# NVlabs/CenterPose

Hardware: NVIDIA H100
Metric: images/sec at 512x512 DLA-34 (dla_34 + DCNv2, 7 heads, decode + PnP) (higher is better)
Workload: dtype tf32x3

## Files before the change

centerpose_b200/csrc/dcn_tma.cu:

```cuda
#include <cuda.h>

#include "common.cuh"
#include "umma_common.cuh"

namespace cp {
namespace {

using namespace umma;

constexpr int DT_BM = 128;
constexpr int DT_THREADS = 512;
constexpr int DT_CS = 16;
constexpr int DT_PH = 8, DT_PW = 16;
constexpr int DT_HALO = 8;
constexpr int DT_SH = DT_PH + 2 * DT_HALO, DT_SW = DT_PW + 2 * DT_HALO;
constexpr uint32_t DT_SLAB_BYTES = DT_SH * DT_SW * DT_CS * 4;
constexpr uint32_t DT_COEF_BYTES = DT_BM * 9 * 16;

struct DcnTmaParams {
  CUtensorMap amap;
  const float* src;
  int srcStride;
  const float* offmask;
  int omStride, mask_is_logit;
// ... 37 lines not shown
    float lh = 0.f, lw = 0.f, mk = 0.f;
    uint32_t pk = 0;
    if (h_im > -1.f && w_im > -1.f && h_im < (float)H && w_im < (float)W) {
      const int h_low = (int)floorf(h_im), w_low = (int)floorf(w_im);
      lh = h_im - (float)h_low;
      lw = w_im - (float)w_low;
      const bool t_ok = h_low >= 0, b_ok = h_low + 1 <= H - 1, l_ok = w_low >= 0, r_ok = w_low + 1 <= W - 1;
      const int hl = t_ok ? h_low : 0, hb = b_ok ? h_low + 1 : H - 1;
      const int wl = l_ok ? w_low : 0, wr = r_ok ? w_low + 1 : W - 1;
      const bool in_slab = (hl >= ys) && (hb < ys + DT_SH) && (wl >= xs) && (wr < xs + DT_SW);
      pk = in_slab ? (uint32_t)((hl - ys) * DT_SW + (wl - xs)) : (uint32_t)((hl << 7) | wl);
      pk |= (uint32_t)(wr - wl) << RB_DX;
      pk |= (uint32_t)(hb - hl) << RB_DY;
      pk |= (uint32_t)((t_ok && l_ok) ? 1 : 0) << (RB_W + 0);
      pk |= (uint32_t)((t_ok && r_ok) ? 1 : 0) << (RB_W + 1);
      pk |= (uint32_t)((b_ok && l_ok) ? 1 : 0) << (RB_W + 2);
      pk |= (uint32_t)((b_ok && r_ok) ? 1 : 0) << (RB_W + 3);
      pk |= (uint32_t)(in_slab ? 1 : 0) << RB_SLAB;
      pk |= 1u << RB_LIVE;
      mk = mm;
    }
    st_shared_v4(dst + (uint32_t)tap * 16u, __float_as_uint(lh), __float_as_uint(lw), __float_as_uint(mk), pk);
  }
}

template <bool X3, int BN>
__global__ void __launch_bounds__(DT_THREADS, 1) dcn_tma_kernel(const __grid_constant__ DcnTmaParams p) {
  extern __shared__ __align__(1024) unsigned char smem[];
  DcnCtl* ctl = reinterpret_cast<DcnCtl*>(smem);
  if (threadIdx.x == 0) griddep_launch_dependents();
  const uint32_t sbase = smem_u32(smem);
  const uint32_t coef0 = sbase + 1024u;
  const uint32_t slabs0 = (coef0 + 2u * DT_COEF_BYTES + 1023u) & ~1023u;
  const uint32_t a_stage = X3 ? 16384u : 8192u;
  const uint32_t atiles0 = slabs0 + 2u * DT_SLAB_BYTES;
  const uint32_t btile_bytes = (uint32_t)BN * 64u * (X3 ? 2u : 1u);
  const uint32_t btiles0 = atiles0 + (uint32_t)p.AH * a_stage;
  const uint32_t drain0 = btiles0 + (uint32_t)p.SB * btile_bytes;

  const int tid = threadIdx.x, warp = tid >> 5, lane = tid & 31;
  const int n_tiles = p.CoutPad / BN;
  const int nslab = p.sps;
  const int KB = nslab * 9;
  const int KB_all = (p.Cin / DT_CS) * 9;
  const int KS_SPLIT = p.ksplit;
  const long long total_tiles = p.total_tiles;

  if (tid == 0) {
    for (int s = 0; s < 2; ++s) {
      mbar_init(smem_u32(&ctl->s_full[s]), 1);
      mbar_init(smem_u32(&ctl->s_empty[s]), 4);
      mbar_init(smem_u32(&ctl->c_full[s]), 4);
      mbar_init(smem_u32(&ctl->c_empty[s]), 4);
    }
    for (int s = 0; s < p.AH; ++s) {
      mbar_init(smem_u32(&ctl->a_full[s]), 4);
      mbar_init(smem_u32(&ctl->a_empty[s]), 2);
    }
    for (int s = 0; s < p.SB; ++s) {
      mbar_init(smem_u32(&ctl->b_full[s]), 1);
      mbar_init(smem_u32(&ctl->b_empty[s]), 2);
    }
    fence_mbar_init();
  }
  __syncthreads();
  if (warp != 1) griddep_wait();

// ... 15 lines not shown
            mbar_arrive_expect_tx(bar, DT_SLAB_BYTES);
            tma_load_4d(slabs0 + (uint32_t)stage * DT_SLAB_BYTES, &p.amap, (s0 + s) * DT_CS, x0 - DT_HALO, y0 - DT_HALO, img,
                        bar);
            if (++stage == 2) {
              stage = 0;
              phase ^= 1u;
            }
          }
        }
      }
      __syncwarp();
    } else if (warp == 1) {
      if (lane == 0) {
        int stage = 0;
        uint32_t phase = 0;
        for (long long tile = blockIdx.x; tile < total_tiles; tile += gridDim.x) {
          const int n_tile = (int)((tile / KS_SPLIT) % n_tiles);
          const unsigned char* wsrc = p.wtiles + ((size_t)n_tile * KB_all + (size_t)(tile % KS_SPLIT) * KB) * btile_bytes;
          for (int kb = 0; kb < KB; ++kb) {
            mbar_wait(smem_u32(&ctl->b_empty[stage]), phase ^ 1u);
            const uint32_t bar = smem_u32(&ctl->b_full[stage]);
            mbar_arrive_expect_tx(bar, btile_bytes);
            bulk_g2s(btiles0 + (uint32_t)stage * btile_bytes, wsrc + (size_t)kb * btile_bytes, btile_bytes, bar);
            if (++stage == p.SB) {
              stage = 0;
              phase ^= 1u;
            }
          }
        }
      }
      __syncwarp();
    }
  } else if (warp >= 8 && warp < 12) {
    const int gt = tid - 256;
    const int row = gt & 127;
    const uint32_t a_row = atiles0 + (uint32_t)(row >> 3) * 512u + (uint32_t)(row & 7) * 64u;
    const uint32_t asw = (uint32_t)(row >> 1) & 3u;
    int ss = 0, cb = 0;
    uint32_t ps = 0, pc = 0;
    uint32_t cnt = 0;
    for (long long tile = blockIdx.x; tile < total_tiles; tile += gridDim.x) {
      const long long m_tile = (tile / KS_SPLIT) / n_tiles;
      const int s0 = (int)(tile % KS_SPLIT) * nslab;
      const int img = (int)(m_tile / p.tiles_per_image);
      mbar_wait(smem_u32(&ctl->c_full[cb]), pc);
      const uint32_t crow = coef0 + (uint32_t)cb * DT_COEF_BYTES + (uint32_t)row * 144u;
      const float* gimg = p.src + (size_t)img * p.H * p.W * p.srcStride;
      int cur = -1;
      uint32_t slab = 0;
      float4 rec_next = ld_shared_v4f(crow);
      for (int kb = 0; kb < KB; ++kb) {
        const int s = kb / 9;
        if (s != cur) {
          if (cur >= 0) {
            __syncwarp();
            if (lane == 0) mbar_arrive(smem_u32(&ctl->s_empty[ss]));
            if (++ss == 2) {
              ss = 0;
              ps ^= 1u;
            }
          }
          mbar_wait(smem_u32(&ctl->s_full[ss]), ps);
          slab = slabs0 + (uint32_t)ss * DT_SLAB_BYTES;
          cur = s;
        }
        const float4 rec = rec_next;
// ... 25 lines not shown
              c2[c] = ld_shared_v4f(b2 ^ ((uint32_t)c << 4));
            }
#pragma unroll
            for (int c = 0; c < 4; ++c) {
              c3[c] = ld_shared_v4f(b3 ^ ((uint32_t)c << 4));
              c4[c] = ld_shared_v4f(b4 ^ ((uint32_t)c << 4));
            }
#pragma unroll
            for (int c = 0; c < 4; ++c) {
              v[c].x = w1 * c1[c].x + w2 * c2[c].x + w3 * c3[c].x + w4 * c4[c].x;
              v[c].y = w1 * c1[c].y + w2 * c2[c].y + w3 * c3[c].y + w4 * c4[c].y;
              v[c].z = w1 * c1[c].z + w2 * c2[c].z + w3 * c3[c].z + w4 * c4[c].z;
              v[c].w = w1 * c1[c].w + w2 * c2[c].w + w3 * c3[c].w + w4 * c4[c].w;
            }
          } else {
            const int hl = (int)((pk >> 7) & 127u), wl = (int)(pk & 127u);
            const float* g = gimg + ((size_t)hl * p.W + wl) * p.srcStride + (s0 + s) * DT_CS;
            const size_t dx = (size_t)((pk >> RB_DX) & 1u) * p.srcStride;
            const size_t dy = (size_t)((pk >> RB_DY) & 1u) * p.W * p.srcStride;
#pragma unroll
            for (int c = 0; c < 4; ++c) {
              const float4 c1 = __ldg(reinterpret_cast<const float4*>(g) + c);
              const float4 c2 = __ldg(reinterpret_cast<const float4*>(g + dx) + c);
              const float4 c3 = __ldg(reinterpret_cast<const float4*>(g + dy) + c);
              const float4 c4 = __ldg(reinterpret_cast<const float4*>(g + dy + dx) + c);
              v[c].x = w1 * c1.x + w2 * c2.x + w3 * c3.x + w4 * c4.x;
              v[c].y = w1 * c1.y + w2 * c2.y + w3 * c3.y + w4 * c4.y;
              v[c].z = w1 * c1.z + w2 * c2.z + w3 * c3.z + w4 * c4.z;
              v[c].w = w1 * c1.w + w2 * c2.w + w3 * c3.w + w4 * c4.w;
            }
          }
        }
        const int sa = (int)(cnt & (uint32_t)(p.AH - 1));
        const uint32_t a_hi = a_row + (uint32_t)sa * a_stage + (asw << 4);
        mbar_wait(smem_u32(&ctl->a_empty[sa]), ((cnt >> (p.AH - 1)) & 1u) ^ 1u);
#pragma unroll
        for (int c = 0; c < 4; ++c) {
          const uint32_t off = (uint32_t)c << 4;
          float4 h;
          h.x = tf32_round(v[c].x);
          h.y = tf32_round(v[c].y);
          h.z = tf32_round(v[c].z);
          h.w = tf32_round(v[c].w);
          st_shared_v4f(a_hi ^ off, h.x, h.y, h.z, h.w);
          if (X3)
            st_shared_v4f((a_hi ^ off) + 8192u, tf32_round(v[c].x - h.x), tf32_round(v[c].y - h.y), tf32_round(v[c].z - h.z),
                          tf32_round(v[c].w - h.w));
        }
        fence_proxy_async_smem();
        __syncwarp();
        if (lane == 0) mbar_arrive(smem_u32(&ctl->a_full[sa]));
        ++cnt;
      }
      __syncwarp();
      if (lane == 0) {
        mbar_arrive(smem_u32(&ctl->s_empty[ss]));
        mbar_arrive(smem_u32(&ctl->c_empty[cb]));
      }
      if (++ss == 2) {
        ss = 0;
        ps ^= 1u;
      }
      if (++cb == 2) {
        cb = 0;
        pc ^= 1u;
      }
    }
  } else {
    asm volatile("setmaxnreg.inc.sync.aligned.u32 168;");
    const int c = warp >= 12 ? 1 : 0, wt = tid & 127;
    float* dstage = reinterpret_cast<float*>(smem + (drain0 - sbase)) + (size_t)c * (DRAIN_STAGE_BYTES / 4);
    EpiParams ep;
    ep.bias = p.bias;
    ep.residual = p.residual;
    ep.resStride = p.resStride;
    ep.relu = p.relu;
    ep.res_after_relu = p.res_after_relu;
    ep.round_tf32 = p.round_tf32;
    ep.out = p.out;
    ep.outStride = p.outStride;
    ep.out_nchw = p.out_nchw;
    ep.Cout = p.Cout;
    ep.CoutPad = p.CoutPad;
    ep.H = p.H;
    ep.W = p.W;
    int cb = 0;
    uint32_t pc = 0;
    auto make_records = [&](long long t) {
      const long long mt = (t / KS_SPLIT) / n_tiles;
      const int im = (int)(mt / p.tiles_per_image);
      const int pt = (int)(mt - (long long)im * p.tiles_per_image);
      const int y0 = (pt / p.tiles_x) * DT_PH, x0 = (pt % p.tiles_x) * DT_PW;
      const int oy = y0 + (wt >> 4), ox = x0 + (wt & 15);
      mbar_wait(smem_u32(&ctl->c_empty[cb]), pc ^ 1u);
      coef_row(p, p.offmask + ((size_t)((size_t)im * p.H + oy) * p.W + ox) * p.omStride, oy, ox, y0 - DT_HALO, x0 - DT_HALO,
               coef0 + (uint32_t)cb * DT_COEF_BYTES + (uint32_t)wt * 144u);
      __syncwarp();
      if (lane == 0) mbar_arrive(smem_u32(&ctl->c_full[cb]));
      if (++cb == 2) {
        cb = 0;
        pc ^= 1u;
      }
    };
    if (c == 0 && (long long)blockIdx.x < total_tiles) make_records(blockIdx.x);
    const uint32_t bar_a_full = smem_u32(&ctl->a_full[0]), bar_a_empty = smem_u32(&ctl->a_empty[0]);
    const uint32_t bar_b_full = smem_u32(&ctl->b_full[0]), bar_b_empty = smem_u32(&ctl->b_empty[0]);
    int sb = 0;
    uint32_t pb = 0, cnt = 0;
    float acc[BN / 2];
    float sums[X3 ? BN / 2 : 1];
#pragma unroll
    for (int j = 0; j < BN / 2; ++j) acc[j] = 0.f;
    for (long long tile = blockIdx.x; tile < total_tiles; tile += gridDim.x) {
      if (c == 0 && tile + gridDim.x < total_tiles) make_records(tile + gridDim.x);
#pragma unroll
      for (int j = 0; j < (X3 ? BN / 2 : 1); ++j) sums[j] = 0.f;
      int gk = 0;
      for (int kbi = 0; kbi < KB; ++kbi, ++cnt) {
        const uint32_t sa = cnt & (uint32_t)(p.AH - 1);
        mbar_wait(bar_a_full + 8u * sa, (cnt >> (p.AH - 1)) & 1u);
        mbar_wait(bar_b_full + 8u * (uint32_t)sb, pb);
        const uint64_t da = make_desc(atiles0 + sa * a_stage + (uint32_t)c * 64u * 64u, DT_CS);
        const uint64_t db = make_desc(btiles0 + (uint32_t)sb * btile_bytes, DT_CS);
        mma_kblock<BN, X3, false, 2>(acc, da, db, 8192u >> 4, ((uint32_t)BN * 64u) >> 4, X3 ? gk == 0 : kbi == 0);
        if (wt == 0) {
          mbar_arrive(bar_a_empty + 8u * sa);
          mbar_arrive(bar_b_empty + 8u * (uint32_t)sb);
        }
        if (++sb == p.SB) {
          sb = 0;
          pb ^= 1u;
        }
        if (X3) {
          if (gk == p.group - 1 || kbi == KB - 1) {
#pragma unroll
            for (int j = 0; j < (X3 ? BN / 2 : 1); ++j) sums[j] += acc[X3 ? j : 0];
            gk = 0;
          } else {
            ++gk;
          }
        }
      }
      const int n_tile = (int)((tile / KS_SPLIT) % n_tiles);
      const long long m_tile = (tile / KS_SPLIT) / n_tiles;
      const int n = (int)(m_tile / p.tiles_per_image);
      const int pt = (int)(m_tile - (long long)n * p.tiles_per_image);
      const int col_end = min(p.Cout, (n_tile + 1) * BN);
      auto fn = [&](int r, int cb0, float (&v)[16]) {
        if (cb0 >= BN) return;
        const int i = c * 64 + r;
        if (KS_SPLIT > 1) {
          float4* part_row = reinterpret_cast<float4*>(p.part) + ((size_t)tile * (BN >> 2) + (cb0 >> 2)) * 128 + i;
#pragma unroll
          for (int q = 0; q < 4; ++q) __stcg(part_row + (size_t)q * 128, make_float4(v[4 * q], v[4 * q + 1], v[4 * q + 2], v[4 * q + 3]));
        } else {
          const int oy = (pt / p.tiles_x) * DT_PH + (i >> 4), ox = (pt % p.tiles_x) * DT_PW + (i & 15);
          const int m = (n * p.H + oy) * p.W + ox;
// ... 28 lines not shown
  if (p.kh != 3 || p.kw != 3 || p.stride != 1 || p.pad != 1) return false;
  if (p.Cin % DT_CS || p.srcStride[0] % 4) return false;
  const int W = p.Win, H = p.Hin;
  if (W > 128 || H > 128 || (W % DT_PW) || (H % DT_PH)) return false;
  return dcn_tma_tile_n(p.CoutPad, x3) != 0;
}

int dcn_tma_encode(const IgemmParams& p, int Bmax, void* map_out) {
  return tma_encode_nhwc_box(p.src[0], p.srcC[0], p.Win, p.Hin, Bmax, p.srcStride[0], DT_CS, DT_SW, DT_SH, 1, map_out);
}

int launch_dcn_tma(const IgemmParams& p, const void* map, const ConvKernel& k, cudaStream_t stream, LaunchInfo* info) {
  const bool x3 = k.x3;
  if (!p.wgt_umma) return fail(CP_ERR_INVALID, "dcn_tma: weight tiles missing");
  if (!dcn_tma_supported(p, x3)) return fail(CP_ERR_INVALID, "dcn_tma: unsupported shape");
  DcnTmaParams q;
  memset(&q, 0, sizeof(q));
  memcpy(&q.amap, map, sizeof(CUtensorMap));
  q.src = p.src[0];
  q.srcStride = p.srcStride[0];
  q.offmask = p.offmask;
  q.omStride = p.omStride;
  q.mask_is_logit = p.mask_is_logit;
  q.B = p.B;
  q.H = p.Hin;
  q.W = p.Win;
  q.Cin = p.Cin;
  q.Cout = p.Cout;
  q.CoutPad = p.CoutPad;
  q.BN = k.BN;
  q.tiles_x = p.Win / DT_PW;
  q.tiles_per_image = q.tiles_x * (p.Hin / DT_PH);
  const long long mn = (long long)q.tiles_per_image * p.B * (p.CoutPad / q.BN);
  const uint32_t a_stage = x3 ? 16384u : 8192u;
  q.group = kX3GroupBlocks * 2;
  const uint32_t btile = (uint32_t)q.BN * 64u * (x3 ? 2u : 1u);
  const size_t budget = 226 * 1024;
  q.AH = 2;
  size_t fixed = 1024 + 2 * (size_t)DT_COEF_BYTES + 1024 + 2 * (size_t)DT_SLAB_BYTES + (size_t)q.AH * a_stage +
                 2 * (size_t)DRAIN_STAGE_BYTES;
  if (fixed + 3 * (size_t)btile > budget) {
    q.AH = 1;
    fixed -= a_stage;
  }
  if (fixed + 2 * (size_t)btile > budget) return fail(CP_ERR_INVALID, "dcn_tma: tile does not fit shared memory");
  q.SB = (int)((budget - fixed) / btile);
  if (q.SB > 8) q.SB = 8;
  q.bias = p.bias;
  q.residual = p.residual;
  q.resStride = p.resStride;
  q.relu = p.relu;
  q.res_after_relu = p.res_after_relu;
  q.out = p.out;
  q.outStride = p.outStride;
  q.out_nchw = p.out_nchw;
  q.round_tf32 = k.round_out;
  q.wtiles = (const unsigned char*)p.wgt_umma;
  const size_t smem = fixed + (size_t)q.SB * btile;
  void (*kern)(DcnTmaParams) = nullptr;
  switch (q.BN) {
    case 16: kern = x3 ? dcn_tma_kernel<true, 16> : dcn_tma_kernel<false, 16>; break;
    case 32: kern = x3 ? dcn_tma_kernel<true, 32> : dcn_tma_kernel<false, 32>; break;
    case 64: kern = x3 ? dcn_tma_kernel<true, 64> : dcn_tma_kernel<false, 64>; break;
    case 128: kern = x3 ? dcn_tma_kernel<true, 128> : dcn_tma_kernel<false, 128>; break;
    default: return fail(CP_ERR_INVALID, "dcn_tma: unsupported N tile");
  }
  static PerDevice<bool, 8> configured;
// ... 30 lines not shown
```

centerpose_b200/csrc/igemm_umma.cu:

```cuda
#include "common.cuh"
#include "umma_common.cuh"

namespace cp {
namespace {

constexpr int UM_BM = 128;
constexpr int UM_PROD_WARPS = 8;
constexpr int UM_THREADS = (UM_PROD_WARPS + 8) * 32;
constexpr uint32_t ROW_BYTES = 128;
constexpr uint32_t A_TILE_BYTES = UM_BM * ROW_BYTES;

using namespace umma;

struct UmmaSmem {
  unsigned long long full[8];
  unsigned long long empty[8];
};

template <int PREC>
struct PrecTraits;
template <>
struct PrecTraits<0> {
  static constexpr int kElems = 64, kChunkCh = 8, kTilesA = 1;
};
template <>
struct PrecTraits<1> {
  static constexpr int kElems = 32, kChunkCh = 4, kTilesA = 2;
};

template <int PREC, int MODE, int BN>
__global__ void __launch_bounds__(UM_THREADS, 1) igemm_umma_kernel(const IgemmParams p, const int STAGES, const int NACC) {
  using T = PrecTraits<PREC>;
  extern __shared__ __align__(1024) unsigned char smem[];
  UmmaSmem* ctl = reinterpret_cast<UmmaSmem*>(smem);
  if (threadIdx.x == 0) griddep_launch_dependents();
  const uint32_t tiles0 = (smem_u32(smem) + 512u + 1023u) & ~1023u;
  const uint32_t b_tile_bytes = (uint32_t)BN * ROW_BYTES * T::kTilesA;
  const uint32_t a_bytes = A_TILE_BYTES * T::kTilesA;
  const uint32_t stage_bytes = a_bytes + b_tile_bytes;

  const int tid = threadIdx.x, warp = tid >> 5;
  const int M = p.B * p.Hout * p.Wout;
  const int n_tiles = p.CoutPad / BN;
  const int n_tile = blockIdx.x % n_tiles;
  const int m0 = (blockIdx.x / n_tiles) * UM_BM;
  const int K = p.kh * p.kw * p.Cin;
  const int KB = (K + T::kElems - 1) / T::kElems;

  if (tid == 0) {
    for (int s = 0; s < STAGES; ++s) {
      mbar_init(smem_u32(&ctl->full[s]), UM_PROD_WARPS * 32 + 1);
      mbar_init(smem_u32(&ctl->empty[s]), 2);
    }
    fence_mbar_init();
  }
  __syncthreads();
  griddep_wait();

  if (warp < UM_PROD_WARPS) {
    {
      const unsigned char* wsrc = reinterpret_cast<const unsigned char*>(p.wgt_umma) + (size_t)n_tile * KB * b_tile_bytes;
      const int r = tid >> 1;
      const int qbase = (tid & 1) * 4;
      const int m = m0 + r;
      const bool valid = m < M;
      int ox = 0, oy = 0, n = 0;
      if (valid) {
        ox = m % p.Wout;
        int t = m / p.Wout;
        oy = t % p.Hout;
        n = t / p.Hout;
      }
// ... 50 lines not shown
                  mk = mm;
                }
              }
              live[qi] = true;
              const int ss = p.srcStride[0];
              const float* base = p.src[0] + (size_t)n * p.Hin * p.Win * ss + c;
#pragma unroll
              for (int h4 = 0; h4 < F4; ++h4) {
                ld[qi][0 * F4 + h4] = __ldg(reinterpret_cast<const float4*>(base + (size_t)o1 * ss) + h4);
                ld[qi][1 * F4 + h4] = __ldg(reinterpret_cast<const float4*>(base + (size_t)o2 * ss) + h4);
                ld[qi][2 * F4 + h4] = __ldg(reinterpret_cast<const float4*>(base + (size_t)o3 * ss) + h4);
                ld[qi][3 * F4 + h4] = __ldg(reinterpret_cast<const float4*>(base + (size_t)o4 * ss) + h4);
              }
            } else {
              const int ky = tap / p.kw, kx = tap - ky * p.kw;
              const int iy = oy * p.stride - p.pad + ky, ix = ox * p.stride - p.pad + kx;
              if (iy >= 0 && iy < p.Hin && ix >= 0 && ix < p.Win) {
                int s = 0, cb = 0;
                while (s + 1 < p.nsrc && c >= cb + p.srcC[s]) {
                  cb += p.srcC[s];
                  ++s;
                }
                const float* sp = p.src[s] + ((size_t)(n * p.Hin + iy) * p.Win + ix) * p.srcStride[s] + (c - cb);
#pragma unroll
                for (int h4 = 0; h4 < F4; ++h4) ld[qi][h4] = __ldg(reinterpret_cast<const float4*>(sp) + h4);
              }
            }
          }
        }
        mbar_wait(smem_u32(&ctl->empty[stage]), phase ^ 1u);
        if (tid == 0) {
          const uint32_t bar = smem_u32(&ctl->full[stage]);
          mbar_arrive_expect_tx(bar, b_tile_bytes);
          bulk_g2s(tiles0 + (uint32_t)stage * stage_bytes + a_bytes, wsrc + (size_t)kb * b_tile_bytes, b_tile_bytes, bar);
        }
        const uint32_t a_hi = tiles0 + (uint32_t)stage * stage_bytes + row_off;
        const uint32_t a_lo = a_hi + A_TILE_BYTES;
#pragma unroll
        for (int qi = 0; qi < 4; ++qi) {
          float v[8];
#pragma unroll
          for (int j = 0; j < 8; ++j) v[j] = 0.f;
          if (MODE == IGEMM_DCN) {
            if (live[qi]) {
#pragma unroll
              for (int h4 = 0; h4 < F4; ++h4) {
                const float4 c1 = ld[qi][0 * F4 + h4], c2 = ld[qi][1 * F4 + h4], c3 = ld[qi][2 * F4 + h4],
                             c4 = ld[qi][3 * F4 + h4];
                v[h4 * 4 + 0] = (w1 * c1.x + w2 * c2.x + w3 * c3.x + w4 * c4.x) * mk;
                v[h4 * 4 + 1] = (w1 * c1.y + w2 * c2.y + w3 * c3.y + w4 * c4.y) * mk;
                v[h4 * 4 + 2] = (w1 * c1.z + w2 * c2.z + w3 * c3.z + w4 * c4.z) * mk;
                v[h4 * 4 + 3] = (w1 * c1.w + w2 * c2.w + w3 * c3.w + w4 * c4.w) * mk;
              }
            }
          } else {
#pragma unroll
            for (int h4 = 0; h4 < F4; ++h4) {
              v[h4 * 4 + 0] = ld[qi][h4].x;
              v[h4 * 4 + 1] = ld[qi][h4].y;
              v[h4 * 4 + 2] = ld[qi][h4].z;
              v[h4 * 4 + 3] = ld[qi][h4].w;
            }
          }
          const uint32_t coff = ((uint32_t)(qbase + qi) ^ sw) << 4;
          if (PREC == 0) {
            st_shared_v4(a_hi + coff, pack_bf16x2(v[0], v[1]), pack_bf16x2(v[2], v[3]), pack_bf16x2(v[4], v[5]),
                         pack_bf16x2(v[6], v[7]));
          } else {
            float h[4], l[4];
#pragma unroll
            for (int j = 0; j < 4; ++j) {
              h[j] = tf32_round(v[j]);
              l[j] = tf32_round(v[j] - h[j]);
            }
            st_shared_v4(a_hi + coff, __float_as_uint(h[0]), __float_as_uint(h[1]), __float_as_uint(h[2]),
                         __float_as_uint(h[3]));
            st_shared_v4(a_lo + coff, __float_as_uint(l[0]), __float_as_uint(l[1]), __float_as_uint(l[2]),
                         __float_as_uint(l[3]));
          }
        }
        fence_proxy_async_smem();
        mbar_arrive(smem_u32(&ctl->full[stage]));
        if (++stage == STAGES) {
          stage = 0;
          phase ^= 1u;
        }
      }
    }

  } else {
    const int c = (warp - UM_PROD_WARPS) >> 2, wt = tid & 127;
    constexpr bool X3 = PREC == 1;
    float acc[BN / 2];
    float sums[X3 ? BN / 2 : 1];
#pragma unroll
    for (int j = 0; j < BN / 2; ++j) acc[j] = 0.f;
#pragma unroll
    for (int j = 0; j < (X3 ? BN / 2 : 1); ++j) sums[j] = 0.f;
    int stage = 0;
    uint32_t phase = 0;
    int gk = 0;
    for (int kb = 0; kb < KB; ++kb) {
      mbar_wait(smem_u32(&ctl->full[stage]), phase);
      const uint32_t a_hi = tiles0 + (uint32_t)stage * stage_bytes;
      const uint64_t da = make_desc(a_hi + (uint32_t)c * 64u * ROW_BYTES, 32), db = make_desc(a_hi + a_bytes, 32);
      mma_kblock<BN, X3, PREC == 0, 4>(acc, da, db, A_TILE_BYTES >> 4, ((uint32_t)BN * ROW_BYTES) >> 4, X3 ? gk == 0 : kb == 0);
      if (wt == 0) mbar_arrive(smem_u32(&ctl->empty[stage]));
      if (++stage == STAGES) {
        stage = 0;
        phase ^= 1u;
      }
      if (X3) {
        if (gk == NACC - 1 || kb == KB - 1) {
#pragma unroll
          for (int j = 0; j < (X3 ? BN / 2 : 1); ++j) sums[j] += acc[X3 ? j : 0];
          gk = 0;
        } else {
          ++gk;
        }
      }
    }
    EpiParams ep;
    ep.bias = p.bias;
    ep.residual = p.residual;
    ep.resStride = p.resStride;
    ep.relu = p.relu;
    ep.res_after_relu = p.res_after_relu;
    ep.round_tf32 = 0;
    ep.out = p.out;
    ep.outStride = p.outStride;
    ep.out_nchw = p.out_nchw;
    ep.Cout = p.Cout;
    ep.CoutPad = p.CoutPad;
    ep.H = p.Hout;
    ep.W = p.Wout;
    const int col_end = min(p.Cout, (n_tile + 1) * BN);
    float* dstage = reinterpret_cast<float*>(smem + (tiles0 - smem_u32(smem)) + (size_t)STAGES * stage_bytes) +
                    (size_t)c * (DRAIN_STAGE_BYTES / 4);
    auto fn = [&](int r, int cb, float (&v)[16]) {
// ... 4 lines not shown
        ox = m % p.Wout;
        const int t = m / p.Wout;
        oy = t % p.Hout;
        n = t / p.Hout;
      }
      if (cb < BN) epilogue_row<16>(ep, v, valid, m, n, oy, ox, n_tile * BN + cb, col_end);
    };
    if constexpr (X3)
      drain_rows<BN>(sums, dstage, wt, 1 + c, fn);
    else
      drain_rows<BN>(acc, dstage, wt, 1 + c, fn);
  }
}

template <int PREC>
__global__ void pack_umma_weight_kernel(const float* __restrict__ src, int ld, int K, int Cout, int BN, int n_tiles,
                                        int KB, unsigned char* __restrict__ dst) {
  using T = PrecTraits<PREC>;
  const size_t total = (size_t)n_tiles * KB * BN * 8;
  for (size_t i = blockIdx.x * (size_t)blockDim.x + threadIdx.x; i < total; i += (size_t)gridDim.x * blockDim.x) {
    const int q = i & 7;
    size_t t = i >> 3;
    const int nr = t % BN;
    t /= BN;
    const int kb = t % KB;
    const int nt = t / KB;
    const int n = nt * BN + nr;
    float v[8];
#pragma unroll
    for (int j = 0; j < 8; ++j) {
      const int k = kb * T::kElems + q * T::kChunkCh + j;
      v[j] = (j < T::kChunkCh && k < K && n < Cout) ? src[(size_t)k * ld + n] : 0.f;
    }
    const size_t tile = ((size_t)nt * KB + kb) * (size_t)BN * ROW_BYTES * T::kTilesA;
    const size_t off = (size_t)(nr >> 3) * 1024 + (size_t)(nr & 7) * 128 + (size_t)((q ^ (nr & 7)) << 4);
    if (PREC == 0) {
      uint4 w;
      w.x = pack_bf16x2(v[0], v[1]);
      w.y = pack_bf16x2(v[2], v[3]);
      w.z = pack_bf16x2(v[4], v[5]);
      w.w = pack_bf16x2(v[6], v[7]);
      *reinterpret_cast<uint4*>(dst + tile + off) = w;
    } else {
      float h[4], l[4];
      for (int j = 0; j < 4; ++j) {
        h[j] = tf32_round(v[j]);
        l[j] = tf32_round(v[j] - h[j]);
      }
      *reinterpret_cast<float4*>(dst + tile + off) = make_float4(h[0], h[1], h[2], h[3]);
      *reinterpret_cast<float4*>(dst + tile + (size_t)BN * ROW_BYTES + off) = make_float4(l[0], l[1], l[2], l[3]);
    }
  }
}

}

int umma_tile_n(int CoutPad, int prec) { return wgmma_tile_n(CoutPad, prec == 1 ? 64 : 128); }

bool umma_supported(const IgemmParams& p, int prec) {
  if (p.mode != IGEMM_NHWC_VEC && p.mode != IGEMM_DCN) return false;
  const int ch = prec == 0 ? 8 : 4;
  if (p.Cin % ch) return false;
  for (int s = 0; s < p.nsrc; ++s)
    if (p.srcC[s] % ch || p.srcStride[s] % 4) return false;
  return umma_tile_n(p.CoutPad, prec) != 0;
}

// ... 18 lines not shown
  else
    pack_umma_weight_kernel<1><<<blocks, 256, 0, s>>>(src, ld, Kreal, Cout, bn, nt, KB, (unsigned char*)dst);
  CP_LAUNCH_CHECK("pack_umma_weight_kernel");
  return CP_OK;
}

template <int PREC, int BN>
static int launch_igemm_umma_bn(const IgemmParams& p, int stages, size_t smem, int nacc, cudaStream_t stream,
                                LaunchInfo* info) {
  void (*kern)(const IgemmParams, const int, const int) =
      (p.mode == IGEMM_DCN) ? igemm_umma_kernel<PREC, IGEMM_DCN, BN> : igemm_umma_kernel<PREC, IGEMM_NHWC_VEC, BN>;
  static PerDevice<bool, 2> configured;
  const int slot = p.mode == IGEMM_DCN ? 1 : 0;
  if (!configured.here(slot)) {
    CP_CUDA_CHECK(cudaFuncSetAttribute(kern, cudaFuncAttributeMaxDynamicSharedMemorySize, 227 * 1024));
    configured.here(slot) = true;
  }
  const int M = p.B * p.Hout * p.Wout;
  dim3 grid((unsigned)((size_t)(p.CoutPad / BN) * ((M + UM_BM - 1) / UM_BM)));
  CP_CUDA_CHECK(launch_kernel(kern, grid, dim3(UM_THREADS), smem, stream, p, stages, nacc));
  CP_LAUNCH_CHECK("igemm_umma_kernel");
  if (info) {
    info->BN = BN;
    info->ksplit = 1;
    info->grid = grid.x;
  }
  return CP_OK;
}

int launch_igemm_umma(const IgemmParams& p, int prec, cudaStream_t stream, LaunchInfo* info) {
  if (!umma_supported(p, prec)) return fail(CP_ERR_INVALID, "igemm_umma: unsupported shape");
  if (!p.wgt_umma) return fail(CP_ERR_INVALID, "igemm_umma: weight tiles missing");
  const int bn = umma_tile_n(p.CoutPad, prec);
  const int tilesA = prec == 0 ? 1 : 2;
  const size_t stage_bytes = (size_t)A_TILE_BYTES * tilesA + (size_t)bn * ROW_BYTES * tilesA;
  const size_t fixed = 512 + 1024 + 2 * (size_t)DRAIN_STAGE_BYTES;
  int stages = (int)((224 * 1024 - fixed) / stage_bytes);
  if (stages > 6) stages = 6;
  if (p.mode == IGEMM_DCN && stages > 2) stages = 2;
  if (stages < 2) return fail(CP_ERR_INVALID, "igemm_umma: tile does not fit shared memory");
  const size_t smem = fixed + stages * stage_bytes;
  const int nacc = prec == 1 ? kX3GroupBlocks : 1;
  if (prec == 0) {
    switch (bn) {
      case 16: return launch_igemm_umma_bn<0, 16>(p, stages, smem, nacc, stream, info);
      case 32: return launch_igemm_umma_bn<0, 32>(p, stages, smem, nacc, stream, info);
      case 64: return launch_igemm_umma_bn<0, 64>(p, stages, smem, nacc, stream, info);
      default: return launch_igemm_umma_bn<0, 128>(p, stages, smem, nacc, stream, info);
    }
  }
  switch (bn) {
    case 16: return launch_igemm_umma_bn<1, 16>(p, stages, smem, nacc, stream, info);
    case 32: return launch_igemm_umma_bn<1, 32>(p, stages, smem, nacc, stream, info);
    default: return launch_igemm_umma_bn<1, 64>(p, stages, smem, nacc, stream, info);
  }
}

}
```

centerpose_b200/csrc/umma_common.cuh:

```cuda
#pragma once
#include <cuda.h>
#include <cuda_runtime.h>
#include <stdint.h>
#include <stdio.h>

namespace cp {
namespace umma {

__device__ __forceinline__ uint32_t smem_u32(const void* p) { return (uint32_t)__cvta_generic_to_shared(p); }

__device__ __forceinline__ void mbar_init(uint32_t bar, uint32_t count) {
  asm volatile("mbarrier.init.shared::cta.b64 [%0], %1;" ::"r"(bar), "r"(count));
}
__device__ __forceinline__ void mbar_arrive(uint32_t bar) {
  asm volatile("mbarrier.arrive.shared::cta.b64 _, [%0];" ::"r"(bar) : "memory");
}
__device__ __forceinline__ void mbar_arrive_expect_tx(uint32_t bar, uint32_t bytes) {
  asm volatile("mbarrier.arrive.expect_tx.shared::cta.b64 _, [%0], %1;" ::"r"(bar), "r"(bytes) : "memory");
}
__device__ __forceinline__ bool mbar_try_wait(uint32_t bar, uint32_t parity) {
  uint32_t ok;
  asm volatile(
      "{\n\t.reg .pred p;\n\tmbarrier.try_wait.parity.shared::cta.b64 p, [%1], %2;\n\tselp.b32 %0, 1, 0, p;\n\t}"
      : "=r"(ok)
// ... 72 lines not shown
      "wgmma.mma_async.sync.aligned.m64n16k16.f32.bf16.bf16 {%0,%1,%2,%3,%4,%5,%6,%7}, %8, %9, p, 1, 1, 0, 0;\n\t}"
      : "+f"(d[0]), "+f"(d[1]), "+f"(d[2]), "+f"(d[3]), "+f"(d[4]), "+f"(d[5]), "+f"(d[6]), "+f"(d[7])
      : "l"(da), "l"(db), "r"(scale_d));
}
template <> __device__ __forceinline__ void wgmma_bf16<32>(float (&d)[16], uint64_t da, uint64_t db, uint32_t scale_d) {
  asm volatile(
      "{\n\t.reg .pred p;\n\tsetp.ne.b32 p, %18, 0;\n\t"
      "wgmma.mma_async.sync.aligned.m64n32k16.f32.bf16.bf16 {%0,%1,%2,%3,%4,%5,%6,%7,%8,%9,%10,%11,%12,%13,%14,%15}, %16, %17, p, 1, 1, 0, 0;\n\t}"
      : "+f"(d[0]), "+f"(d[1]), "+f"(d[2]), "+f"(d[3]), "+f"(d[4]), "+f"(d[5]), "+f"(d[6]), "+f"(d[7]), "+f"(d[8]), "+f"(d[9]), "+f"(d[10]), "+f"(d[11]), "+f"(d[12]), "+f"(d[13]), "+f"(d[14]), "+f"(d[15])
      : "l"(da), "l"(db), "r"(scale_d));
}
template <> __device__ __forceinline__ void wgmma_bf16<64>(float (&d)[32], uint64_t da, uint64_t db, uint32_t scale_d) {
  asm volatile(
      "{\n\t.reg .pred p;\n\tsetp.ne.b32 p, %34, 0;\n\t"
      "wgmma.mma_async.sync.aligned.m64n64k16.f32.bf16.bf16 {%0,%1,%2,%3,%4,%5,%6,%7,%8,%9,%10,%11,%12,%13,%14,%15,%16,%17,%18,%19,%20,%21,%22,%23,%24,%25,%26,%27,%28,%29,%30,%31}, %32, %33, p, 1, 1, 0, 0;\n\t}"
      : "+f"(d[0]), "+f"(d[1]), "+f"(d[2]), "+f"(d[3]), "+f"(d[4]), "+f"(d[5]), "+f"(d[6]), "+f"(d[7]), "+f"(d[8]), "+f"(d[9]), "+f"(d[10]), "+f"(d[11]), "+f"(d[12]), "+f"(d[13]), "+f"(d[14]), "+f"(d[15]), "+f"(d[16]), "+f"(d[17]), "+f"(d[18]), "+f"(d[19]), "+f"(d[20]), "+f"(d[21]), "+f"(d[22]), "+f"(d[23]), "+f"(d[24]), "+f"(d[25]), "+f"(d[26]), "+f"(d[27]), "+f"(d[28]), "+f"(d[29]), "+f"(d[30]), "+f"(d[31])
      : "l"(da), "l"(db), "r"(scale_d));
}
template <> __device__ __forceinline__ void wgmma_bf16<128>(float (&d)[64], uint64_t da, uint64_t db, uint32_t scale_d) {
  asm volatile(
      "{\n\t.reg .pred p;\n\tsetp.ne.b32 p, %66, 0;\n\t"
      "wgmma.mma_async.sync.aligned.m64n128k16.f32.bf16.bf16 {%0,%1,%2,%3,%4,%5,%6,%7,%8,%9,%10,%11,%12,%13,%14,%15,%16,%17,%18,%19,%20,%21,%22,%23,%24,%25,%26,%27,%28,%29,%30,%31,%32,%33,%34,%35,%36,%37,%38,%39,%40,%41,%42,%43,%44,%45,%46,%47,%48,%49,%50,%51,%52,%53,%54,%55,%56,%57,%58,%59,%60,%61,%62,%63}, %64, %65, p, 1, 1, 0, 0;\n\t}"
      : "+f"(d[0]), "+f"(d[1]), "+f"(d[2]), "+f"(d[3]), "+f"(d[4]), "+f"(d[5]), "+f"(d[6]), "+f"(d[7]), "+f"(d[8]), "+f"(d[9]), "+f"(d[10]), "+f"(d[11]), "+f"(d[12]), "+f"(d[13]), "+f"(d[14]), "+f"(d[15]), "+f"(d[16]), "+f"(d[17]), "+f"(d[18]), "+f"(d[19]), "+f"(d[20]), "+f"(d[21]), "+f"(d[22]), "+f"(d[23]), "+f"(d[24]), "+f"(d[25]), "+f"(d[26]), "+f"(d[27]), "+f"(d[28]), "+f"(d[29]), "+f"(d[30]), "+f"(d[31]), "+f"(d[32]), "+f"(d[33]), "+f"(d[34]), "+f"(d[35]), "+f"(d[36]), "+f"(d[37]), "+f"(d[38]), "+f"(d[39]), "+f"(d[40]), "+f"(d[41]), "+f"(d[42]), "+f"(d[43]), "+f"(d[44]), "+f"(d[45]), "+f"(d[46]), "+f"(d[47]), "+f"(d[48]), "+f"(d[49]), "+f"(d[50]), "+f"(d[51]), "+f"(d[52]), "+f"(d[53]), "+f"(d[54]), "+f"(d[55]), "+f"(d[56]), "+f"(d[57]), "+f"(d[58]), "+f"(d[59]), "+f"(d[60]), "+f"(d[61]), "+f"(d[62]), "+f"(d[63])
      : "l"(da), "l"(db), "r"(scale_d));
}
template <> __device__ __forceinline__ void wgmma_bf16<256>(float (&d)[128], uint64_t da, uint64_t db, uint32_t scale_d) {
  asm volatile(
      "{\n\t.reg .pred p;\n\tsetp.ne.b32 p, %130, 0;\n\t"
      "wgmma.mma_async.sync.aligned.m64n256k16.f32.bf16.bf16 {%0,%1,%2,%3,%4,%5,%6,%7,%8,%9,%10,%11,%12,%13,%14,%15,%16,%17,%18,%19,%20,%21,%22,%23,%24,%25,%26,%27,%28,%29,%30,%31,%32,%33,%34,%35,%36,%37,%38,%39,%40,%41,%42,%43,%44,%45,%46,%47,%48,%49,%50,%51,%52,%53,%54,%55,%56,%57,%58,%59,%60,%61,%62,%63,%64,%65,%66,%67,%68,%69,%70,%71,%72,%73,%74,%75,%76,%77,%78,%79,%80,%81,%82,%83,%84,%85,%86,%87,%88,%89,%90,%91,%92,%93,%94,%95,%96,%97,%98,%99,%100,%101,%102,%103,%104,%105,%106,%107,%108,%109,%110,%111,%112,%113,%114,%115,%116,%117,%118,%119,%120,%121,%122,%123,%124,%125,%126,%127}, %128, %129, p, 1, 1, 0, 0;\n\t}"
      : "+f"(d[0]), "+f"(d[1]), "+f"(d[2]), "+f"(d[3]), "+f"(d[4]), "+f"(d[5]), "+f"(d[6]), "+f"(d[7]), "+f"(d[8]), "+f"(d[9]), "+f"(d[10]), "+f"(d[11]), "+f"(d[12]), "+f"(d[13]), "+f"(d[14]), "+f"(d[15]), "+f"(d[16]), "+f"(d[17]), "+f"(d[18]), "+f"(d[19]), "+f"(d[20]), "+f"(d[21]), "+f"(d[22]), "+f"(d[23]), "+f"(d[24]), "+f"(d[25]), "+f"(d[26]), "+f"(d[27]), "+f"(d[28]), "+f"(d[29]), "+f"(d[30]), "+f"(d[31]), "+f"(d[32]), "+f"(d[33]), "+f"(d[34]), "+f"(d[35]), "+f"(d[36]), "+f"(d[37]), "+f"(d[38]), "+f"(d[39]), "+f"(d[40]), "+f"(d[41]), "+f"(d[42]), "+f"(d[43]), "+f"(d[44]), "+f"(d[45]), "+f"(d[46]), "+f"(d[47]), "+f"(d[48]), "+f"(d[49]), "+f"(d[50]), "+f"(d[51]), "+f"(d[52]), "+f"(d[53]), "+f"(d[54]), "+f"(d[55]), "+f"(d[56]), "+f"(d[57]), "+f"(d[58]), "+f"(d[59]), "+f"(d[60]), "+f"(d[61]), "+f"(d[62]), "+f"(d[63]), "+f"(d[64]), "+f"(d[65]), "+f"(d[66]), "+f"(d[67]), "+f"(d[68]), "+f"(d[69]), "+f"(d[70]), "+f"(d[71]), "+f"(d[72]), "+f"(d[73]), "+f"(d[74]), "+f"(d[75]), "+f"(d[76]), "+f"(d[77]), "+f"(d[78]), "+f"(d[79]), "+f"(d[80]), "+f"(d[81]), "+f"(d[82]), "+f"(d[83]), "+f"(d[84]), "+f"(d[85]), "+f"(d[86]), "+f"(d[87]), "+f"(d[88]), "+f"(d[89]), "+f"(d[90]), "+f"(d[91]), "+f"(d[92]), "+f"(d[93]), "+f"(d[94]), "+f"(d[95]), "+f"(d[96]), "+f"(d[97]), "+f"(d[98]), "+f"(d[99]), "+f"(d[100]), "+f"(d[101]), "+f"(d[102]), "+f"(d[103]), "+f"(d[104]), "+f"(d[105]), "+f"(d[106]), "+f"(d[107]), "+f"(d[108]), "+f"(d[109]), "+f"(d[110]), "+f"(d[111]), "+f"(d[112]), "+f"(d[113]), "+f"(d[114]), "+f"(d[115]), "+f"(d[116]), "+f"(d[117]), "+f"(d[118]), "+f"(d[119]), "+f"(d[120]), "+f"(d[121]), "+f"(d[122]), "+f"(d[123]), "+f"(d[124]), "+f"(d[125]), "+f"(d[126]), "+f"(d[127])
      : "l"(da), "l"(db), "r"(scale_d));
}

template <int BN, bool X3, bool BF16, int KS>
__device__ __forceinline__ void mma_kblock(float (&acc)[BN / 2], uint64_t da, uint64_t db, uint32_t a_lo, uint32_t b_lo,
                                           bool fresh) {
  wg_fence();
#pragma unroll
  for (int ks = 0; ks < KS; ++ks) {
    const uint32_t sd = (fresh && ks == 0) ? 0u : 1u;
    if (X3) {
      wgmma_tf32<BN>(acc, da + a_lo + 2u * ks, db + 2u * ks, sd);
      wgmma_tf32<BN>(acc, da + 2u * ks, db + b_lo + 2u * ks, 1u);
    } else if (BF16) {
      wgmma_bf16<BN>(acc, da + 2u * ks, db + 2u * ks, sd);
    } else {
      wgmma_tf32<BN>(acc, da + 2u * ks, db + 2u * ks, sd);
    }
  }
  if (X3) {
#pragma unroll
    for (int ks = 0; ks < KS; ++ks) wgmma_tf32<BN>(acc, da + 2u * ks, db + 2u * ks, 1u);
  }
  wg_commit();
  wg_wait<0>();
}

__device__ __forceinline__ float tf32_round(float x) {
  return __uint_as_float((__float_as_uint(x) + 0x1000u) & 0xffffe000u);
}
__device__ __forceinline__ uint32_t pack_bf16x2(float a, float b) {
  uint32_t r;
  asm("cvt.rn.bf16x2.f32 %0, %1, %2;" : "=r"(r) : "f"(b), "f"(a));
  return r;
}
__device__ __forceinline__ void st_shared_v4(uint32_t addr, uint32_t a, uint32_t b, uint32_t c, uint32_t d) {
  asm volatile("st.shared.v4.b32 [%0], {%1, %2, %3, %4};" ::"r"(addr), "r"(a), "r"(b), "r"(c), "r"(d) : "memory");
}
__device__ __forceinline__ void st_shared_v4f(uint32_t addr, float a, float b, float c, float d) {
  asm volatile("st.shared.v4.f32 [%0], {%1, %2, %3, %4};" ::"r"(addr), "f"(a), "f"(b), "f"(c), "f"(d) : "memory");
}
__device__ __forceinline__ float4 ld_shared_v4f(uint32_t addr) {
  float4 v;
  asm volatile("ld.shared.v4.f32 {%0,%1,%2,%3}, [%4];" : "=f"(v.x), "=f"(v.y), "=f"(v.z), "=f"(v.w) : "r"(addr) : "memory");
  return v;
}

__device__ __forceinline__ void tma_load_4d(uint32_t dst, const CUtensorMap* map, int c0, int c1, int c2, int c3, uint32_t bar) {
  asm volatile(
      "cp.async.bulk.tensor.4d.shared::cluster.global.tile.mbarrier::complete_tx::bytes [%0], [%1, {%2, %3, %4, %5}], [%6];" ::"r"(dst),
      "l"(map), "r"(c0), "r"(c1), "r"(c2), "r"(c3), "r"(bar)
      : "memory");
}
__device__ __forceinline__ void tma_load_2d(uint32_t dst, const CUtensorMap* map, int c0, int c1, uint32_t bar) {
  asm volatile("cp.async.bulk.tensor.2d.shared::cluster.global.tile.mbarrier::complete_tx::bytes [%0], [%1, {%2, %3}], [%4];" ::"r"(dst),
               "l"(map), "r"(c0), "r"(c1), "r"(bar)
               : "memory");
}
__device__ __forceinline__ bool elect_one() {
  uint32_t pred;
  asm volatile("{\n\t.reg .pred p;\n\telect.sync _|p, 0xffffffff;\n\tselp.u32 %0, 1, 0, p;\n\t}" : "=r"(pred));
  return pred != 0;
}
// ... 125 lines not shown
```

Measured before the change: 654.0.

## Split tf32x3 A operand in registers and feed wgmma from registers

Producers now store the raw fp32 A tile once instead of separate hi and lo tf32 tiles, which halves A-stage shared memory and producer stores. The MMA warpgroups load A with ldmatrix, split it into hi and lo in registers, and issue register-sourced wgmma for the three-product tf32x3 scheme. Register budgets shift between roles to make room: producers drop to 120 and consumers rise to 176. The cost is extra ALU work and register pressure in the consumer warps. Freed shared memory may allow more pipeline stages.

Result: faster. 679.1, median of 6 (+3.8%).

```diff
diff --git a/centerpose_b200/csrc/dcn_tma.cu b/centerpose_b200/csrc/dcn_tma.cu
--- a/centerpose_b200/csrc/dcn_tma.cu
+++ b/centerpose_b200/csrc/dcn_tma.cu
@@ -93,7 +93,7 @@
   const uint32_t sbase = smem_u32(smem);
   const uint32_t coef0 = sbase + 1024u;
   const uint32_t slabs0 = (coef0 + 2u * DT_COEF_BYTES + 1023u) & ~1023u;
-  const uint32_t a_stage = X3 ? 16384u : 8192u;
+  const uint32_t a_stage = 8192u;
   const uint32_t atiles0 = slabs0 + 2u * DT_SLAB_BYTES;
   const uint32_t btile_bytes = (uint32_t)BN * 64u * (X3 ? 2u : 1u);
   const uint32_t btiles0 = atiles0 + (uint32_t)p.AH * a_stage;
@@ -175,6 +175,7 @@
       __syncwarp();
     }
   } else if (warp >= 8 && warp < 12) {
+    asm volatile("setmaxnreg.dec.sync.aligned.u32 120;");
     const int gt = tid - 256;
     const int row = gt & 127;
     const uint32_t a_row = atiles0 + (uint32_t)(row >> 3) * 512u + (uint32_t)(row & 7) * 64u;
@@ -266,20 +267,15 @@
           }
         }
         const int sa = (int)(cnt & (uint32_t)(p.AH - 1));
-        const uint32_t a_hi = a_row + (uint32_t)sa * a_stage + (asw << 4);
+        const uint32_t a_dst = a_row + (uint32_t)sa * a_stage + (asw << 4);
         mbar_wait(smem_u32(&ctl->a_empty[sa]), ((cnt >> (p.AH - 1)) & 1u) ^ 1u);
 #pragma unroll
         for (int c = 0; c < 4; ++c) {
           const uint32_t off = (uint32_t)c << 4;
-          float4 h;
-          h.x = tf32_round(v[c].x);
-          h.y = tf32_round(v[c].y);
-          h.z = tf32_round(v[c].z);
-          h.w = tf32_round(v[c].w);
-          st_shared_v4f(a_hi ^ off, h.x, h.y, h.z, h.w);
           if (X3)
-            st_shared_v4f((a_hi ^ off) + 8192u, tf32_round(v[c].x - h.x), tf32_round(v[c].y - h.y), tf32_round(v[c].z - h.z),
-                          tf32_round(v[c].w - h.w));
+            st_shared_v4f(a_dst ^ off, v[c].x, v[c].y, v[c].z, v[c].w);
+          else
+            st_shared_v4f(a_dst ^ off, tf32_round(v[c].x), tf32_round(v[c].y), tf32_round(v[c].z), tf32_round(v[c].w));
         }
         fence_proxy_async_smem();
         __syncwarp();
@@ -301,7 +297,7 @@
       }
     }
   } else {
-    asm volatile("setmaxnreg.inc.sync.aligned.u32 168;");
+    asm volatile("setmaxnreg.inc.sync.aligned.u32 176;");
     const int c = warp >= 12 ? 1 : 0, wt = tid & 127;
     float* dstage = reinterpret_cast<float*>(smem + (drain0 - sbase)) + (size_t)c * (DRAIN_STAGE_BYTES / 4);
     EpiParams ep;
@@ -354,9 +350,12 @@
         const uint32_t sa = cnt & (uint32_t)(p.AH - 1);
         mbar_wait(bar_a_full + 8u * sa, (cnt >> (p.AH - 1)) & 1u);
         mbar_wait(bar_b_full + 8u * (uint32_t)sb, pb);
-        const uint64_t da = make_desc(atiles0 + sa * a_stage + (uint32_t)c * 64u * 64u, DT_CS);
+        const uint32_t a_tile = atiles0 + sa * a_stage + (uint32_t)c * 64u * 64u;
         const uint64_t db = make_desc(btiles0 + (uint32_t)sb * btile_bytes, DT_CS);
-        mma_kblock<BN, X3, false, 2>(acc, da, db, 8192u >> 4, ((uint32_t)BN * 64u) >> 4, X3 ? gk == 0 : kbi == 0);
+        if (X3)
+          mma_kblock_x3<BN, 2>(acc, a_tile, wt, db, ((uint32_t)BN * 64u) >> 4, gk == 0);
+        else
+          mma_kblock<BN, false, false, 2>(acc, make_desc(a_tile, DT_CS), db, 0, 0, kbi == 0);
         if (wt == 0) {
           mbar_arrive(bar_a_empty + 8u * sa);
           mbar_arrive(bar_b_empty + 8u * (uint32_t)sb);
@@ -451,7 +450,7 @@
   q.tiles_x = p.Win / DT_PW;
   q.tiles_per_image = q.tiles_x * (p.Hin / DT_PH);
   const long long mn = (long long)q.tiles_per_image * p.B * (p.CoutPad / q.BN);
-  const uint32_t a_stage = x3 ? 16384u : 8192u;
+  const uint32_t a_stage = 8192u;
   q.group = kX3GroupBlocks * 2;
   const uint32_t btile = (uint32_t)q.BN * 64u * (x3 ? 2u : 1u);
   const size_t budget = 226 * 1024;
diff --git a/centerpose_b200/csrc/igemm_umma.cu b/centerpose_b200/csrc/igemm_umma.cu
--- a/centerpose_b200/csrc/igemm_umma.cu
+++ b/centerpose_b200/csrc/igemm_umma.cu
@@ -21,11 +21,11 @@
 struct PrecTraits;
 template <>
 struct PrecTraits<0> {
-  static constexpr int kElems = 64, kChunkCh = 8, kTilesA = 1;
+  static constexpr int kElems = 64, kChunkCh = 8, kTilesB = 1;
 };
 template <>
 struct PrecTraits<1> {
-  static constexpr int kElems = 32, kChunkCh = 4, kTilesA = 2;
+  static constexpr int kElems = 32, kChunkCh = 4, kTilesB = 2;
 };
 
 template <int PREC, int MODE, int BN>
@@ -35,9 +35,8 @@
   UmmaSmem* ctl = reinterpret_cast<UmmaSmem*>(smem);
   if (threadIdx.x == 0) griddep_launch_dependents();
   const uint32_t tiles0 = (smem_u32(smem) + 512u + 1023u) & ~1023u;
-  const uint32_t b_tile_bytes = (uint32_t)BN * ROW_BYTES * T::kTilesA;
-  const uint32_t a_bytes = A_TILE_BYTES * T::kTilesA;
-  const uint32_t stage_bytes = a_bytes + b_tile_bytes;
+  const uint32_t b_tile_bytes = (uint32_t)BN * ROW_BYTES * T::kTilesB;
+  const uint32_t stage_bytes = A_TILE_BYTES + b_tile_bytes;
 
   const int tid = threadIdx.x, warp = tid >> 5;
   const int M = p.B * p.Hout * p.Wout;
@@ -154,10 +153,9 @@
         if (tid == 0) {
           const uint32_t bar = smem_u32(&ctl->full[stage]);
           mbar_arrive_expect_tx(bar, b_tile_bytes);
-          bulk_g2s(tiles0 + (uint32_t)stage * stage_bytes + a_bytes, wsrc + (size_t)kb * b_tile_bytes, b_tile_bytes, bar);
-        }
-        const uint32_t a_hi = tiles0 + (uint32_t)stage * stage_bytes + row_off;
-        const uint32_t a_lo = a_hi + A_TILE_BYTES;
+          bulk_g2s(tiles0 + (uint32_t)stage * stage_bytes + A_TILE_BYTES, wsrc + (size_t)kb * b_tile_bytes, b_tile_bytes, bar);
+        }
+        const uint32_t a_dst = tiles0 + (uint32_t)stage * stage_bytes + row_off;
 #pragma unroll
         for (int qi = 0; qi < 4; ++qi) {
           float v[8];
@@ -185,21 +183,11 @@
             }
           }
           const uint32_t coff = ((uint32_t)(qbase + qi) ^ sw) << 4;
-          if (PREC == 0) {
-            st_shared_v4(a_hi + coff, pack_bf16x2(v[0], v[1]), pack_bf16x2(v[2], v[3]), pack_bf16x2(v[4], v[5]),
+          if (PREC == 0)
+            st_shared_v4(a_dst + coff, pack_bf16x2(v[0], v[1]), pack_bf16x2(v[2], v[3]), pack_bf16x2(v[4], v[5]),
                          pack_bf16x2(v[6], v[7]));
-          } else {
-            float h[4], l[4];
-#pragma unroll
-            for (int j = 0; j < 4; ++j) {
-              h[j] = tf32_round(v[j]);
-              l[j] = tf32_round(v[j] - h[j]);
-            }
-            st_shared_v4(a_hi + coff, __float_as_uint(h[0]), __float_as_uint(h[1]), __float_as_uint(h[2]),
-                         __float_as_uint(h[3]));
-            st_shared_v4(a_lo + coff, __float_as_uint(l[0]), __float_as_uint(l[1]), __float_as_uint(l[2]),
-                         __float_as_uint(l[3]));
-          }
+          else
+            st_shared_v4f(a_dst + coff, v[0], v[1], v[2], v[3]);
         }
         fence_proxy_async_smem();
         mbar_arrive(smem_u32(&ctl->full[stage]));
@@ -224,9 +212,12 @@
     int gk = 0;
     for (int kb = 0; kb < KB; ++kb) {
       mbar_wait(smem_u32(&ctl->full[stage]), phase);
-      const uint32_t a_hi = tiles0 + (uint32_t)stage * stage_bytes;
-      const uint64_t da = make_desc(a_hi + (uint32_t)c * 64u * ROW_BYTES, 32), db = make_desc(a_hi + a_bytes, 32);
-      mma_kblock<BN, X3, PREC == 0, 4>(acc, da, db, A_TILE_BYTES >> 4, ((uint32_t)BN * ROW_BYTES) >> 4, X3 ? gk == 0 : kb == 0);
+      const uint32_t a_tile = tiles0 + (uint32_t)stage * stage_bytes + (uint32_t)c * 64u * ROW_BYTES;
+      const uint64_t db = make_desc(tiles0 + (uint32_t)stage * stage_bytes + A_TILE_BYTES, 32);
+      if (X3)
+        mma_kblock_x3<BN, 4>(acc, a_tile, wt, db, ((uint32_t)BN * ROW_BYTES) >> 4, gk == 0);
+      else
+        mma_kblock<BN, false, true, 4>(acc, make_desc(a_tile, 32), db, 0, 0, kb == 0);
       if (wt == 0) mbar_arrive(smem_u32(&ctl->empty[stage]));
       if (++stage == STAGES) {
         stage = 0;
@@ -297,7 +288,7 @@
       const int k = kb * T::kElems + q * T::kChunkCh + j;
       v[j] = (j < T::kChunkCh && k < K && n < Cout) ? src[(size_t)k * ld + n] : 0.f;
     }
-    const size_t tile = ((size_t)nt * KB + kb) * (size_t)BN * ROW_BYTES * T::kTilesA;
+    const size_t tile = ((size_t)nt * KB + kb) * (size_t)BN * ROW_BYTES * T::kTilesB;
     const size_t off = (size_t)(nr >> 3) * 1024 + (size_t)(nr & 7) * 128 + (size_t)((q ^ (nr & 7)) << 4);
     if (PREC == 0) {
       uint4 w;
@@ -382,8 +373,7 @@
   if (!umma_supported(p, prec)) return fail(CP_ERR_INVALID, "igemm_umma: unsupported shape");
   if (!p.wgt_umma) return fail(CP_ERR_INVALID, "igemm_umma: weight tiles missing");
   const int bn = umma_tile_n(p.CoutPad, prec);
-  const int tilesA = prec == 0 ? 1 : 2;
-  const size_t stage_bytes = (size_t)A_TILE_BYTES * tilesA + (size_t)bn * ROW_BYTES * tilesA;
+  const size_t stage_bytes = (size_t)A_TILE_BYTES + (size_t)bn * ROW_BYTES * (prec == 0 ? 1 : 2);
   const size_t fixed = 512 + 1024 + 2 * (size_t)DRAIN_STAGE_BYTES;
   int stages = (int)((224 * 1024 - fixed) / stage_bytes);
   if (stages > 6) stages = 6;
diff --git a/centerpose_b200/csrc/umma_common.cuh b/centerpose_b200/csrc/umma_common.cuh
--- a/centerpose_b200/csrc/umma_common.cuh
+++ b/centerpose_b200/csrc/umma_common.cuh
@@ -128,6 +128,37 @@
       : "l"(da), "l"(db), "r"(scale_d));
 }
 
+template <int N>
+__device__ __forceinline__ void wgmma_tf32_rs(float (&d)[N / 2], const uint32_t (&a)[4], uint64_t db, uint32_t scale_d);
+template <> __device__ __forceinline__ void wgmma_tf32_rs<16>(float (&d)[8], const uint32_t (&a)[4], uint64_t db, uint32_t scale_d) {
+  asm volatile(
+      "{\n\t.reg .pred p;\n\tsetp.ne.b32 p, %13, 0;\n\t"
+      "wgmma.mma_async.sync.aligned.m64n16k8.f32.tf32.tf32 {%0,%1,%2,%3,%4,%5,%6,%7}, {%8,%9,%10,%11}, %12, p, 1, 1;\n\t}"
+      : "+f"(d[0]), "+f"(d[1]), "+f"(d[2]), "+f"(d[3]), "+f"(d[4]), "+f"(d[5]), "+f"(d[6]), "+f"(d[7])
+      : "r"(a[0]), "r"(a[1]), "r"(a[2]), "r"(a[3]), "l"(db), "r"(scale_d));
+}
+template <> __device__ __forceinline__ void wgmma_tf32_rs<32>(float (&d)[16], const uint32_t (&a)[4], uint64_t db, uint32_t scale_d) {
+  asm volatile(
+      "{\n\t.reg .pred p;\n\tsetp.ne.b32 p, %21, 0;\n\t"
+      "wgmma.mma_async.sync.aligned.m64n32k8.f32.tf32.tf32 {%0,%1,%2,%3,%4,%5,%6,%7,%8,%9,%10,%11,%12,%13,%14,%15}, {%16,%17,%18,%19}, %20, p, 1, 1;\n\t}"
+      : "+f"(d[0]), "+f"(d[1]), "+f"(d[2]), "+f"(d[3]), "+f"(d[4]), "+f"(d[5]), "+f"(d[6]), "+f"(d[7]), "+f"(d[8]), "+f"(d[9]), "+f"(d[10]), "+f"(d[11]), "+f"(d[12]), "+f"(d[13]), "+f"(d[14]), "+f"(d[15])
+      : "r"(a[0]), "r"(a[1]), "r"(a[2]), "r"(a[3]), "l"(db), "r"(scale_d));
+}
+template <> __device__ __forceinline__ void wgmma_tf32_rs<64>(float (&d)[32], const uint32_t (&a)[4], uint64_t db, uint32_t scale_d) {
+  asm volatile(
+      "{\n\t.reg .pred p;\n\tsetp.ne.b32 p, %37, 0;\n\t"
+      "wgmma.mma_async.sync.aligned.m64n64k8.f32.tf32.tf32 {%0,%1,%2,%3,%4,%5,%6,%7,%8,%9,%10,%11,%12,%13,%14,%15,%16,%17,%18,%19,%20,%21,%22,%23,%24,%25,%26,%27,%28,%29,%30,%31}, {%32,%33,%34,%35}, %36, p, 1, 1;\n\t}"
+      : "+f"(d[0]), "+f"(d[1]), "+f"(d[2]), "+f"(d[3]), "+f"(d[4]), "+f"(d[5]), "+f"(d[6]), "+f"(d[7]), "+f"(d[8]), "+f"(d[9]), "+f"(d[10]), "+f"(d[11]), "+f"(d[12]), "+f"(d[13]), "+f"(d[14]), "+f"(d[15]), "+f"(d[16]), "+f"(d[17]), "+f"(d[18]), "+f"(d[19]), "+f"(d[20]), "+f"(d[21]), "+f"(d[22]), "+f"(d[23]), "+f"(d[24]), "+f"(d[25]), "+f"(d[26]), "+f"(d[27]), "+f"(d[28]), "+f"(d[29]), "+f"(d[30]), "+f"(d[31])
+      : "r"(a[0]), "r"(a[1]), "r"(a[2]), "r"(a[3]), "l"(db), "r"(scale_d));
+}
+template <> __device__ __forceinline__ void wgmma_tf32_rs<128>(float (&d)[64], const uint32_t (&a)[4], uint64_t db, uint32_t scale_d) {
+  asm volatile(
+      "{\n\t.reg .pred p;\n\tsetp.ne.b32 p, %69, 0;\n\t"
+      "wgmma.mma_async.sync.aligned.m64n128k8.f32.tf32.tf32 {%0,%1,%2,%3,%4,%5,%6,%7,%8,%9,%10,%11,%12,%13,%14,%15,%16,%17,%18,%19,%20,%21,%22,%23,%24,%25,%26,%27,%28,%29,%30,%31,%32,%33,%34,%35,%36,%37,%38,%39,%40,%41,%42,%43,%44,%45,%46,%47,%48,%49,%50,%51,%52,%53,%54,%55,%56,%57,%58,%59,%60,%61,%62,%63}, {%64,%65,%66,%67}, %68, p, 1, 1;\n\t}"
+      : "+f"(d[0]), "+f"(d[1]), "+f"(d[2]), "+f"(d[3]), "+f"(d[4]), "+f"(d[5]), "+f"(d[6]), "+f"(d[7]), "+f"(d[8]), "+f"(d[9]), "+f"(d[10]), "+f"(d[11]), "+f"(d[12]), "+f"(d[13]), "+f"(d[14]), "+f"(d[15]), "+f"(d[16]), "+f"(d[17]), "+f"(d[18]), "+f"(d[19]), "+f"(d[20]), "+f"(d[21]), "+f"(d[22]), "+f"(d[23]), "+f"(d[24]), "+f"(d[25]), "+f"(d[26]), "+f"(d[27]), "+f"(d[28]), "+f"(d[29]), "+f"(d[30]), "+f"(d[31]), "+f"(d[32]), "+f"(d[33]), "+f"(d[34]), "+f"(d[35]), "+f"(d[36]), "+f"(d[37]), "+f"(d[38]), "+f"(d[39]), "+f"(d[40]), "+f"(d[41]), "+f"(d[42]), "+f"(d[43]), "+f"(d[44]), "+f"(d[45]), "+f"(d[46]), "+f"(d[47]), "+f"(d[48]), "+f"(d[49]), "+f"(d[50]), "+f"(d[51]), "+f"(d[52]), "+f"(d[53]), "+f"(d[54]), "+f"(d[55]), "+f"(d[56]), "+f"(d[57]), "+f"(d[58]), "+f"(d[59]), "+f"(d[60]), "+f"(d[61]), "+f"(d[62]), "+f"(d[63])
+      : "r"(a[0]), "r"(a[1]), "r"(a[2]), "r"(a[3]), "l"(db), "r"(scale_d));
+}
+
 template <int BN, bool X3, bool BF16, int KS>
 __device__ __forceinline__ void mma_kblock(float (&acc)[BN / 2], uint64_t da, uint64_t db, uint32_t a_lo, uint32_t b_lo,
                                            bool fresh) {
@@ -155,6 +186,47 @@
 __device__ __forceinline__ float tf32_round(float x) {
   return __uint_as_float((__float_as_uint(x) + 0x1000u) & 0xffffe000u);
 }
+__device__ __forceinline__ void ldsm_x4(uint32_t (&r)[4], uint32_t addr) {
+  asm volatile("ldmatrix.sync.aligned.m8n8.x4.shared.b16 {%0, %1, %2, %3}, [%4];"
+               : "=r"(r[0]), "=r"(r[1]), "=r"(r[2]), "=r"(r[3])
+               : "r"(addr));
+}
+
+template <int BN, int KS>
+__device__ __forceinline__ void mma_kblock_x3(float (&acc)[BN / 2], uint32_t a_tile, int wt, uint64_t db, uint32_t b_lo,
+                                              bool fresh) {
+  const uint32_t lane = (uint32_t)wt & 31u;
+  const uint32_t row = (uint32_t)(wt >> 5) * 16u + (lane & 7u) + ((lane >> 3) & 1u) * 8u;
+  const uint32_t a_row = a_tile + row * (32u * KS);
+  const uint32_t x = ((lane >> 4) << 4) ^ ((a_row >> 3) & (KS == 4 ? 0x70u : 0x30u));
+  uint32_t hi[KS][4], lo[KS][4];
+#pragma unroll
+  for (int ks = 0; ks < KS; ++ks) {
+    ldsm_x4(hi[ks], a_row + (((uint32_t)ks << 5) ^ x));
+#pragma unroll
+    for (int j = 0; j < 4; ++j) {
+      const float v = __uint_as_float(hi[ks][j]);
+      const float h = tf32_round(v);
+      lo[ks][j] = __float_as_uint(tf32_round(v - h));
+      hi[ks][j] = __float_as_uint(h);
+    }
+  }
+  wg_fence();
+#pragma unroll
+  for (int ks = 0; ks < KS; ++ks) {
+    wgmma_tf32_rs<BN>(acc, lo[ks], db + 2u * ks, (fresh && ks == 0) ? 0u : 1u);
+    wgmma_tf32_rs<BN>(acc, hi[ks], db + b_lo + 2u * ks, 1u);
+  }
+#pragma unroll
+  for (int ks = 0; ks < KS; ++ks) wgmma_tf32_rs<BN>(acc, hi[ks], db + 2u * ks, 1u);
+  wg_commit();
+  wg_wait<0>();
+#pragma unroll
+  for (int ks = 0; ks < KS; ++ks)
+#pragma unroll
+    for (int j = 0; j < 4; ++j) asm volatile("" : "+r"(hi[ks][j]), "+r"(lo[ks][j]));
+}
+
 __device__ __forceinline__ uint32_t pack_bf16x2(float a, float b) {
   uint32_t r;
   asm("cvt.rn.bf16x2.f32 %0, %1, %2;" : "=r"(r) : "f"(b), "f"(a));
```
